# deepomicslab/PALACE

Measured on AMD Instinct MI355X. Metric: contigs/sec eref+generate_graph+matching, 1M-contig synth, 1/2/4/8 GPU, higher is better.
Workload: dtype u32

## Files before the change

include/palace_hip.h:

```cpp
#ifndef PALACE_HIP_H
#define PALACE_HIP_H

#include <stddef.h>
#include <stdint.h>

#ifdef __cplusplus
extern "C" {
#endif

#define PALACE_OK 0
#define PALACE_EINVAL (-1)
#define PALACE_EHIP (-2)
#define PALACE_ENOMEM (-3)
#define PALACE_ESTATE (-4)

typedef struct palace_ctx palace_ctx;

const char *palace_last_error(void);
const char *palace_version(void);

int palace_ctx_create(int device, palace_ctx **out);
int palace_ctx_create_prio(int device, int high_priority, palace_ctx **out);
int palace_ctx_create_on_stream(int device, void *hip_stream, palace_ctx **out);
int palace_ctx_destroy(palace_ctx *ctx);
// ... 21 lines not shown
int palace_eref_set_coder(palace_ctx *ctx, const uint8_t header400[400]);

int palace_eref_index_refs(palace_ctx *ctx, const uint8_t *d_bases, const int64_t *d_offsets,
                           int64_t n_refs, uint32_t *d_out, const int64_t *d_out_offsets);

int palace_eref_table_reset(palace_ctx *ctx);
int palace_eref_reserve(palace_ctx *ctx, int64_t total_bases);
int palace_eref_count_reads(palace_ctx *ctx, const uint8_t *d_bases, const int64_t *d_offsets,
                            int64_t n_reads, const uint8_t *d_keep, int64_t total_bases);

size_t palace_eref_packed_bytes(int64_t n_positions);
int palace_eref_pack_reads(palace_ctx *ctx, const uint8_t *d_bases, const int64_t *d_offsets, int64_t n_reads,
                           const uint8_t *d_keep, int64_t total_bases, uint32_t *d_p0, uint32_t *d_p1, uint32_t *d_u);
int palace_eref_count_reads_packed(palace_ctx *ctx, const uint32_t *d_p0, const uint32_t *d_p1, const uint32_t *d_u,
                                   int64_t n_positions, int64_t n_reads_hint);

int palace_eref_set_count_mode(palace_ctx *ctx, int mode, int64_t bucket_cap);
int palace_eref_set_key_buckets(palace_ctx *ctx, const uint32_t mask128[4]);
int palace_eref_set_option(palace_ctx *ctx, const char *name, int64_t value);

int palace_eref_scan_refs(palace_ctx *ctx, const uint8_t *d_bases, const int64_t *d_offsets,
                          int64_t n_refs, int64_t total_bases, int one_min, int three_min,
                          int32_t *d_rows);

typedef struct palace_eref_probe_index palace_eref_probe_index;
int palace_eref_probe_index_build(palace_ctx *ctx, const uint8_t *d_bases, const int64_t *d_offsets, int64_t n_refs,
                                  int64_t total_bases, palace_eref_probe_index **out);
int palace_eref_probe_index_free(palace_ctx *ctx, palace_eref_probe_index *ix);
int palace_eref_scan_refs_indexed(palace_ctx *ctx, const palace_eref_probe_index *ix, const uint8_t *d_bases,
                                  const int64_t *d_offsets, int64_t n_refs, int64_t total_bases, int one_min,
                                  int three_min, int32_t *d_rows);

int palace_eref_attach_probe_index(palace_ctx *ctx, const palace_eref_probe_index *ix);

int palace_eref_entry_layout(const palace_eref_probe_index *ix, size_t *counts_bytes, size_t *hits_bytes);
int palace_eref_entry_buffers_attach(palace_ctx *ctx, palace_eref_probe_index *ix, void *d_counts, void *d_hits);
int palace_eref_entry_buffers(const palace_eref_probe_index *ix, void **d_counts, void **d_hits);
int palace_eref_entry_hits_from_counts(palace_ctx *ctx, const palace_eref_probe_index *ix, const void *d_parts, int n_parts, size_t part_stride,
                                       size_t off, size_t bytes);
int palace_eref_entry_hits_complete(palace_ctx *ctx, const palace_eref_probe_index *ix, int64_t keys_counted);
int palace_eref_entry_counts_valid(const palace_ctx *ctx, const palace_eref_probe_index *ix);


int palace_eref_table_planes(palace_ctx *ctx, void **d_planes3, size_t *bytes_per_plane);
int palace_eref_table_attach(palace_ctx *ctx, void *const d_planes3[3]);
int palace_eref_table_invalidate(palace_ctx *ctx);
// ... 568 lines not shown
```

palace_amd/capi.py:

```python
from __future__ import annotations

import ctypes as C
import os
import subprocess

import numpy as np

_HERE = os.path.dirname(os.path.abspath(__file__))
SO_PATH = os.environ.get("PALACE_HIP_SO") or os.path.join(_HERE, "libpalace_hip.so")
_LIB = None


class PalaceError(RuntimeError):
    pass


def build(force: bool = False) -> str:
    args = ["make", "-C", os.path.join(_HERE, "csrc")]
    if force:
        subprocess.run(args + ["clean"], check=True, stdout=subprocess.DEVNULL)
    subprocess.run(args, check=True, stdout=subprocess.DEVNULL)
    return SO_PATH


# ... 105 lines not shown
    "palace_host_alloc": [C.c_void_p, C.c_size_t, C.POINTER(C.c_void_p)],
    "palace_host_free": [C.c_void_p, C.c_void_p],
    "palace_d2h_async": [C.c_void_p, C.c_void_p, C.c_void_p, C.c_size_t],
    "palace_h2d_async": [C.c_void_p, C.c_void_p, C.c_void_p, C.c_size_t],
    "palace_mark_wait": [C.c_void_p, C.c_int],
    "palace_mark_wait_for": [C.c_void_p, C.c_int, C.c_double],
    "palace_wait_for_mark": [C.c_void_p, C.c_void_p, C.c_int],
    "palace_timer_begin": [C.c_void_p],
    "palace_timer_end": [C.c_void_p, C.POINTER(C.c_float)],
    "palace_mark": [C.c_void_p, C.c_int],
    "palace_mark_elapsed": [C.c_void_p, C.c_int, C.c_int, C.POINTER(C.c_float)],
    "palace_eref_set_coder": [C.c_void_p, C.c_void_p],
    "palace_eref_index_refs": [C.c_void_p, C.c_void_p, C.c_void_p, C.c_int64, C.c_void_p, C.c_void_p],
    "palace_eref_table_reset": [C.c_void_p],
    "palace_eref_reserve": [C.c_void_p, C.c_int64],
    "palace_eref_count_reads": [C.c_void_p, C.c_void_p, C.c_void_p, C.c_int64, C.c_void_p, C.c_int64],
    "palace_eref_pack_reads": [C.c_void_p, C.c_void_p, C.c_void_p, C.c_int64, C.c_void_p, C.c_int64, C.c_void_p, C.c_void_p, C.c_void_p],
    "palace_eref_count_reads_packed": [C.c_void_p, C.c_void_p, C.c_void_p, C.c_void_p, C.c_int64, C.c_int64],
    "palace_eref_set_count_mode": [C.c_void_p, C.c_int, C.c_int64],
    "palace_eref_set_key_buckets": [C.c_void_p, C.c_void_p],
    "palace_eref_set_option": [C.c_void_p, C.c_char_p, C.c_int64],
    "palace_eref_scan_refs": [C.c_void_p, C.c_void_p, C.c_void_p, C.c_int64, C.c_int64, C.c_int, C.c_int,
                              C.c_void_p],
    "palace_eref_probe_index_build": [C.c_void_p, C.c_void_p, C.c_void_p, C.c_int64, C.c_int64, C.POINTER(C.c_void_p)],
    "palace_eref_attach_probe_index": [C.c_void_p, C.c_void_p],
    "palace_eref_entry_layout": [C.c_void_p, C.POINTER(C.c_size_t), C.POINTER(C.c_size_t)],
    "palace_eref_entry_buffers_attach": [C.c_void_p, C.c_void_p, C.c_void_p, C.c_void_p],
    "palace_eref_entry_buffers": [C.c_void_p, C.POINTER(C.c_void_p), C.POINTER(C.c_void_p)],
    "palace_eref_entry_hits_from_counts": [C.c_void_p, C.c_void_p, C.c_void_p, C.c_int, C.c_size_t, C.c_size_t, C.c_size_t],
    "palace_eref_entry_hits_complete": [C.c_void_p, C.c_void_p, C.c_int64],
    "palace_eref_entry_counts_valid": [C.c_void_p, C.c_void_p],
    "palace_eref_probe_index_free": [C.c_void_p, C.c_void_p],
    "palace_eref_scan_refs_indexed": [C.c_void_p, C.c_void_p, C.c_void_p, C.c_void_p, C.c_int64, C.c_int64, C.c_int, C.c_int,
                                      C.c_void_p],
    "palace_eref_table_planes": [C.c_void_p, C.POINTER(C.c_void_p), C.POINTER(C.c_size_t)],
    "palace_eref_table_attach": [C.c_void_p, C.POINTER(C.c_void_p)],
    "palace_eref_table_invalidate": [C.c_void_p],
    "palace_eref_table_merge_slices": [C.c_void_p, C.c_void_p, C.c_int, C.c_size_t, C.c_size_t],
    "palace_eref_table_merge_slices_packed": [C.c_void_p, C.c_void_p, C.c_int, C.c_size_t, C.c_size_t],
    "palace_eref_table_pack_low": [C.c_void_p, C.c_void_p],
    "palace_eref_plane_pack": [C.c_void_p, C.c_void_p, C.c_void_p, C.c_void_p, C.c_int64, C.c_void_p],
    "palace_eref_plane_unpack": [C.c_void_p, C.c_void_p, C.c_void_p, C.c_void_p, C.c_int64, C.c_void_p],
    "palace_eref_table_lookup": [C.c_void_p, C.c_void_p, C.c_int64, C.c_void_p],
    "palace_eref_table_popcounts": [C.c_void_p, C.POINTER(C.c_uint64)],
    "palace_graph_classify": [C.c_void_p, C.POINTER(BamCols), C.c_void_p, C.c_int32, C.c_void_p, C.c_void_p,
                              C.c_void_p, C.c_int64, C.POINTER(GraphParams), C.c_int64, C.c_void_p, C.c_void_p,
# ... 1811 lines not shown
```

palace_amd/csrc/eref_common.hpp:

```cpp
#pragma once
#include "common.hpp"

#ifdef PALACE_STAMPS
extern __device__ unsigned long long palace_stamp_buf[8 * 65536];
#define STAMP(arr, i) do { if (arr) (arr)[i] = __builtin_amdgcn_s_memrealtime(); } while (0)
#else
#define STAMP(arr, i) do { } while (0)
#endif

namespace palace {

struct BaseBits {
    bool p0, p1, p2, ok;
};

__device__ __forceinline__ BaseBits classify(uint32_t ch)
{
    const uint32_t x = ch & 0xDFu;
    const uint32_t d = x - 0x41u;
    const bool ok = d < 20u && ((0x80045u >> d) & 1u);
    const uint32_t c = x >> 1;
    return BaseBits{!(c & 1u), !(c & 2u), !((c ^ (c >> 1)) & 1u), ok};
}

// ... 178 lines not shown
static inline KeyBuckets ctx_buckets(const palace_ctx *ctx)
{
    KeyBuckets k;
    for (int i = 0; i < 4; i++) k.m[i] = ctx->key_buckets[i];
    return k;
}

constexpr size_t kTouchedBytes = 8192 + 256;
struct CountPlan {
    int64_t slab_bases_max = 0, n_slabs = 0, n_chunks = 0;
    DensityCaps caps1{}, caps2{};
    size_t cur1_bytes = 0, cur2_bytes = 0, buf1_bytes = 0, buf2_bytes = 0, words_bytes = 0;
    size_t total() const { return cur1_bytes + buf1_bytes + cur2_bytes + kTouchedBytes + 5 * words_bytes + buf2_bytes; }
};
constexpr int64_t kRegions = static_cast<int64_t>(kL1Buckets) * kL1Replicas;

struct CountBufs {
    unsigned int *cursor2 = nullptr, *touched = nullptr, *cursor1 = nullptr;
    unsigned long long *words = nullptr;
    uint32_t *buf1 = nullptr;
    uint16_t *buf2 = nullptr;
};

struct ScanBuffers {
    int64_t *tile_pre, *word_pre;
    uint64_t *any_w, *all_w, *good_w;
    uint32_t *any_p, *all_p;
    uint8_t *need, *active;
    uint8_t *hit_bytes;
    uint8_t *ehits[kSets];
    int64_t max_tiles, max_words;
};
int scan_buffers(palace_ctx *ctx, const int64_t *d_offsets, int64_t n_refs, int64_t total_bases, ScanBuffers *b, bool with_hit_bytes = false,
                 const size_t *ehits_bytes = nullptr);

}

struct palace_eref_probe_index {
    int64_t n_refs = 0, total_bases = 0;
    palace::CoderMasks masks{};
    unsigned long long n_entries[palace::kSets] = {0, 0, 0, 0};
    unsigned long long *first = nullptr;
    uint16_t *keys16[palace::kSets] = {nullptr, nullptr, nullptr, nullptr};
    uint32_t *eix[3] = {nullptr, nullptr, nullptr};
    uint32_t *pos_s = nullptr;
    uint8_t *ehits_own[palace::kSets] = {nullptr, nullptr, nullptr, nullptr};
    size_t ehits_own_bytes = 0;
    uint8_t *sent_bytes_own = nullptr;
    uint8_t *ecnt_own[palace::kSets] = {nullptr, nullptr, nullptr, nullptr};
    size_t entry_hits_bytes = 0;
    size_t set_at[palace::kSets] = {0, 0, 0, 0};
// ... 15 lines not shown
```

palace_amd/csrc/eref_scan.hip:

```cpp
#include "eref_common.hpp"

namespace palace {

__global__ __launch_bounds__(1024) void seq_prefix_kernel(const int64_t *__restrict__ offsets,
                                                          int64_t n, int64_t *__restrict__ tile_pre,
                                                          int64_t *__restrict__ word_pre)
{
    __shared__ int64_t s_t[1024], s_w[1024];
    const int t = threadIdx.x;
    const int64_t per = (n + 1023) / 1024;
    const int64_t a = min(n, t * per), b = min(n, a + per);
    int64_t st = 0, sw = 0;
    for (int64_t r = a; r < b; r++) {
        int64_t len = offsets[r + 1] - offsets[r];
        st += (len + kTilePos - 1) / kTilePos;
        sw += (len + 63) / 64;
    }
    s_t[t] = st;
    s_w[t] = sw;
    __syncthreads();
    for (int d = 1; d < 1024; d <<= 1) {
        int64_t vt = (t >= d) ? s_t[t - d] : 0, vw = (t >= d) ? s_w[t - d] : 0;
        __syncthreads();
        s_t[t] += vt;
        s_w[t] += vw;
        __syncthreads();
    }
    int64_t rt = s_t[t] - st, rw = s_w[t] - sw;
    for (int64_t r = a; r < b; r++) {
        int64_t len = offsets[r + 1] - offsets[r];
// ... 263 lines not shown
                at++;
            }
        }
        __syncthreads();
        const uint32_t n = min(n_list, static_cast<uint32_t>(kScatterList));
        const unsigned long long eb = base * 128;
        constexpr int kUn = 4;
        for (uint32_t j0 = threadIdx.x; j0 < n; j0 += kUn * kScatterThreads) {
            uint32_t p[kUn];
#pragma unroll
            for (int u = 0; u < kUn; u++) {
                const uint32_t j = j0 + u * kScatterThreads;
                p[u] = j < n ? pos[eb + list[j]] : ~0u;
            }
#pragma unroll
            for (int u = 0; u < kUn; u++)
                if (p[u] != ~0u) hit(p[u]);
        }
        __syncthreads();
    }
}

constexpr int kRefThreads = 1024;
__global__ __launch_bounds__(kRefThreads) void eref_need_kernel(const int64_t *__restrict__ offsets, int64_t n_refs,
                                                        const int64_t *__restrict__ word_pre,
                                                        const uint64_t *__restrict__ c0_words,
                                                        uint32_t *__restrict__ c0_pre, uint64_t *__restrict__ cand_words,
                                                        uint32_t *__restrict__ cand_pre, int three_min,
                                                        uint8_t *__restrict__ need, uint8_t *__restrict__ active,
                                                        int64_t r_lo, int64_t r_hi)
{
    const int64_t r = blockIdx.x;
    if (r >= n_refs) return;
    if (r < r_lo || r >= r_hi) { if (threadIdx.x == 0) active[r] = 0; return; }
    const int64_t len = offsets[r + 1] - offsets[r];
    const int64_t n_words = (len + 63) / 64, w0 = word_pre[r];
    const uint64_t *A = c0_words + w0;
    uint32_t *PA = c0_pre + w0, *PC = cand_pre + w0;
    uint64_t *C = cand_words + w0;
    const int t = threadIdx.x, lane = t & 63, wv = t >> 6;
    constexpr int kWaves = kRefThreads / 64;
    __shared__ uint32_t s_part[kWaves];
    __shared__ uint32_t carry;
    auto block_prefix = [&](const uint64_t *W, uint32_t *P) {
        if (t == 0) carry = 0;
        __syncthreads();
        for (int64_t base = 0; base < n_words; base += kRefThreads) {
            const int64_t w = base + t;
            const uint32_t c = (w < n_words) ? __popcll(W[w]) : 0;
            uint32_t inc = c;
#pragma unroll
            for (int d = 1; d < 64; d <<= 1) {
                uint32_t u = __shfl_up(inc, d);
                if (lane >= d) inc += u;
            }
            if (lane == 63) s_part[wv] = inc;
            __syncthreads();
            uint32_t o = carry;
            for (int k = 0; k < wv; k++) o += s_part[k];
            if (w < n_words) P[w] = o + inc - c;
            __syncthreads();
            if (t == kRefThreads - 1) carry = o + inc;
            __syncthreads();
        }
    };
    {
        bool dense = false;
        for (int64_t g = t; g * 8 < n_words; g += kRefThreads) {
            uint32_t c = 0;
#pragma unroll
            for (int k = 0; k < 8; k++) c += (g * 8 + k < n_words) ? __popcll(A[g * 8 + k]) : 0;
            dense |= 2 * static_cast<int>(c) >= three_min;
        }
        const bool live = __syncthreads_or(dense);
        if (!live) {
            if (t == 0) active[r] = 0;
            return;
        }
        if (t == 0) active[r] = 1;
    }
    block_prefix(A, PA);
    __threadfence_block();
    __syncthreads();
    for (int64_t w = wv; w < n_words; w += kWaves) {
        const int64_t j = w * 64 + lane;
        bool cand = false;
        if (j < len) {
            uint32_t c = prefix_count(A, PA, j);
            if (j >= 500) c -= prefix_count(A, PA, j - 500);
            cand = static_cast<int>(c) >= three_min;
        }
        const uint64_t g = __ballot(cand);
        if (lane == 0) C[w] = g;
    }
    __threadfence_block();
    __syncthreads();
    block_prefix(C, PC);
    __threadfence_block();
    __syncthreads();
    if (carry == 0) {
        if (t == 0) active[r] = 0;
        return;
    }
    for (int64_t w = t; w < n_words; w += kRefThreads) {
        const int64_t hi = min(len - 1, w * 64 + 63 + 499);
        uint32_t upto = prefix_count(C, PC, hi);
        uint32_t before = w ? prefix_count(C, PC, w * 64 - 1) : 0u;
        need[w0 + w] = upto > before;
    }
}

__global__ __launch_bounds__(kRefThreads) void eref_window_kernel(const int64_t *__restrict__ offsets,
                                                                  int64_t n_refs,
                                                                  const int64_t *__restrict__ word_pre,
                                                                  const uint64_t *__restrict__ any_words,
                                                                  const uint64_t *__restrict__ all_words,
                                                                  uint32_t *__restrict__ any_pre,
                                                                  uint32_t *__restrict__ all_pre,
                                                                  uint64_t *__restrict__ good_words,
                                                                  int one_min, int three_min,
                                                                  const uint8_t *__restrict__ active,
                                                                  int32_t *__restrict__ rows)
{
    const int64_t r = blockIdx.x;
    if (r >= n_refs) return;
    const int64_t len = offsets[r + 1] - offsets[r];
    if (!active[r]) {
        if (threadIdx.x == 0) { rows[4 * r + 0] = 0; rows[4 * r + 1] = 0; rows[4 * r + 2] = static_cast<int>(len); rows[4 * r + 3] = 0; }
        return;
    }
    const int64_t n_words = (len + 63) / 64, w0 = word_pre[r];
    const uint64_t *A = any_words + w0, *T = all_words + w0;
    uint32_t *PA = any_pre + w0, *PT = all_pre + w0;
    uint64_t *G = good_words + w0;
    const int t = threadIdx.x, lane = t & 63, wv = t >> 6;
    constexpr int kWaves = kRefThreads / 64;

    __shared__ uint32_t s_a[kWaves], s_t[kWaves];
    __shared__ uint32_t carry_a, carry_t;
    if (t == 0) { carry_a = 0; carry_t = 0; }
    __syncthreads();
    for (int64_t base = 0; base < n_words; base += kRefThreads) {
        int64_t w = base + t;
        uint32_t ca = (w < n_words) ? __popcll(A[w]) : 0, ct = (w < n_words) ? __popcll(T[w]) : 0;
        uint32_t ia = ca, it = ct;
#pragma unroll
        for (int d = 1; d < 64; d <<= 1) {
            uint32_t ua = __shfl_up(ia, d), ut = __shfl_up(it, d);
            if (lane >= d) { ia += ua; it += ut; }
        }
        if (lane == 63) { s_a[wv] = ia; s_t[wv] = it; }
        __syncthreads();
        uint32_t oa = carry_a, ot = carry_t;
        for (int k = 0; k < wv; k++) { oa += s_a[k]; ot += s_t[k]; }
        if (w < n_words) { PA[w] = oa + ia - ca; PT[w] = ot + it - ct; }
        __syncthreads();
        if (t == kRefThreads - 1) { carry_a = oa + ia; carry_t = ot + it; }
        __syncthreads();
    }
    __threadfence_block();
    __syncthreads();

    for (int64_t w = wv; w < n_words; w += kWaves) {
        int64_t j = w * 64 + lane;
        bool good = false;
        if (j < len) {
            uint32_t one = prefix_count(A, PA, j), three = prefix_count(T, PT, j);
            if (j >= 500) { one -= prefix_count(A, PA, j - 500); three -= prefix_count(T, PT, j - 500); }
            good = static_cast<int>(one) >= one_min && static_cast<int>(three) >= three_min;
        }
        uint64_t g = __ballot(good);
        if (lane == 0) G[w] = g;
    }
    __threadfence_block();
    __syncthreads();

    constexpr int kMaxEdges = 1024;
    __shared__ uint32_t edge[kMaxEdges];
    __shared__ unsigned int n_edge;
    if (t == 0) n_edge = 0;
    __syncthreads();
    for (int64_t w = t; w <= n_words; w += kRefThreads) {
        const uint64_t g = (w < n_words) ? G[w] : 0;
        const uint64_t prev_bit = w ? (G[w - 1] >> 63) : 0;
        uint64_t x = g ^ ((g << 1) | prev_bit);
        while (x) {
            const int b = __ffsll(static_cast<long long>(x)) - 1;
            x &= x - 1;
            const unsigned int at = atomicAdd(&n_edge, 1u);
            if (at < kMaxEdges) edge[at] = (static_cast<uint32_t>(w * 64 + b) << 1) | static_cast<uint32_t>((g >> b) & 1);
        }
    }
    __syncthreads();
    if (t == 0) {
        int frag = 0, el = 0, start = 0, prev_end = 0;
        const int ilen = static_cast<int>(len);
        auto on_edge = [&](int j, bool rising) {
            if (rising) {
                start = max(1, j - 1000);
            } else {
                int end = min(ilen, j + 1000);
                if (frag > 0 && start - prev_end < 500) { el += end - prev_end; }
                else { frag++; el += end - start; }
                prev_end = end;
            }
        };
        if (n_edge <= kMaxEdges) {
            const int n = static_cast<int>(n_edge);
            for (int i = 1; i < n; i++) {
                const uint32_t e = edge[i];
                int k = i - 1;
                while (k >= 0 && edge[k] > e) { edge[k + 1] = edge[k]; k--; }
                edge[k + 1] = e;
            }
            for (int i = 0; i < n; i++) on_edge(static_cast<int>(edge[i] >> 1), edge[i] & 1u);
        } else {
            uint64_t prev_bit = 0;
            for (int64_t w = 0; w <= n_words; w++) {
                uint64_t g = (w < n_words) ? G[w] : 0;
                uint64_t x = g ^ ((g << 1) | prev_bit);
                while (x) {
                    int b = __ffsll(static_cast<long long>(x)) - 1;
                    x &= x - 1;
                    on_edge(static_cast<int>(w * 64 + b), (g >> b) & 1);
                }
                prev_bit = g >> 63;
            }
        }
        rows[4 * r + 0] = frag;
        rows[4 * r + 1] = el;
        rows[4 * r + 2] = ilen;
        rows[4 * r + 3] = 0;
    }
}

}

using namespace palace;

extern "C" {

static int launch_prefix(palace_ctx *ctx, const int64_t *d_offsets, int64_t n, int64_t *tile_pre, int64_t *word_pre)
{
    hipLaunchKernelGGL(seq_prefix_kernel, dim3(1), dim3(1024), 0, ctx->stream, d_offsets, n, tile_pre, word_pre);
    PALACE_HIP_TRY(hipGetLastError());
    return PALACE_OK;
}

int palace_eref_index_refs(palace_ctx *ctx, const uint8_t *d_bases, const int64_t *d_offsets,
                           int64_t n_refs, uint32_t *d_out, const int64_t *d_out_offsets)
{
    PALACE_REQUIRE(ctx && n_refs >= 0, "bad argument");
    if (!ctx->coder_set) { set_error("palace_eref_index_refs: coder not set"); return PALACE_ESTATE; }
    if (n_refs == 0) return PALACE_OK;
    PALACE_REQUIRE(d_bases && d_offsets && d_out && d_out_offsets, "null device pointer");
    PALACE_HIP_TRY(hipSetDevice(ctx->device));
    int64_t h_off[2];
    PALACE_HIP_TRY(hipMemcpyAsync(&h_off[0], d_offsets, 8, hipMemcpyDeviceToHost, ctx->stream));
    PALACE_HIP_TRY(hipMemcpyAsync(&h_off[1], d_offsets + n_refs, 8, hipMemcpyDeviceToHost, ctx->stream));
    PALACE_HIP_TRY(hipStreamSynchronize(ctx->stream));
    int64_t total = h_off[1] - h_off[0];
    PALACE_REQUIRE(total >= 0, "offsets not ascending");
    size_t pre_bytes = align_up((n_refs + 1) * 8, 256);
    int rc = ensure_workspace(ctx, 2 * pre_bytes);
    if (rc) return rc;
    char *ws = static_cast<char *>(ctx->ws.ptr);
    int64_t *tile_pre = reinterpret_cast<int64_t *>(ws), *word_pre = reinterpret_cast<int64_t *>(ws + pre_bytes);
// ... 5 lines not shown
                       d_bases, d_offsets, n_refs, tile_pre, word_pre, ctx->masks,
                       static_cast<const uint32_t *>(nullptr), static_cast<uint64_t *>(nullptr),
                       static_cast<uint64_t *>(nullptr), d_out, d_out_offsets, static_cast<const uint8_t *>(nullptr),
                       static_cast<const uint8_t *>(nullptr));
    PALACE_HIP_TRY(hipGetLastError());
    return PALACE_OK;
}

}

namespace palace {
int scan_buffers(palace_ctx *ctx, const int64_t *d_offsets, int64_t n_refs, int64_t total_bases, ScanBuffers *b, bool with_hit_bytes,
                 const size_t *ehits_bytes)
{
    b->max_tiles = total_bases / kTilePos + n_refs;
    b->max_words = total_bases / 64 + n_refs + 1;
    PALACE_REQUIRE(b->max_tiles < (1ll << 31), "too many tiles for one launch");
    const size_t pre_bytes = align_up((n_refs + 1) * 8, 256);
    const size_t w64 = align_up(b->max_words * 8, 256), w32 = align_up(b->max_words * 4, 256);
    const size_t w8 = align_up(b->max_words, 256);
    const size_t hb = with_hit_bytes ? align_up(static_cast<size_t>(b->max_words) * (64 / kSentinelStride), 256) : 0;
    size_t eb[kSets] = {0, 0, 0, 0}, eb_all = 0;
    for (int k = 0; k < kSets; k++) { eb[k] = ehits_bytes && ehits_bytes[k] ? align_up(ehits_bytes[k] + 16, 256) : 0; eb_all += eb[k]; }
    int rc = ensure_workspace(ctx, 2 * pre_bytes + 3 * w64 + 2 * w32 + w8 + align_up(n_refs + 1, 256) + hb + eb_all);
    if (rc) return rc;
    char *ws = static_cast<char *>(ctx->ws.ptr);
    b->tile_pre = reinterpret_cast<int64_t *>(ws); ws += pre_bytes;
    b->word_pre = reinterpret_cast<int64_t *>(ws); ws += pre_bytes;
    b->any_w = reinterpret_cast<uint64_t *>(ws); ws += w64;
    b->all_w = reinterpret_cast<uint64_t *>(ws); ws += w64;
    b->good_w = reinterpret_cast<uint64_t *>(ws); ws += w64;
    b->any_p = reinterpret_cast<uint32_t *>(ws); ws += w32;
    b->all_p = reinterpret_cast<uint32_t *>(ws); ws += w32;
    b->need = reinterpret_cast<uint8_t *>(ws); ws += w8;
    b->active = reinterpret_cast<uint8_t *>(ws); ws += align_up(n_refs + 1, 256);
    b->hit_bytes = with_hit_bytes ? reinterpret_cast<uint8_t *>(ws) : nullptr; ws += hb;
    for (int k = 0; k < kSets; k++) { b->ehits[k] = eb[k] ? reinterpret_cast<uint8_t *>(ws) : nullptr; ws += eb[k]; }
    return launch_prefix(ctx, d_offsets, n_refs, b->tile_pre, b->word_pre);
}
}

namespace {
int scan_tail(palace_ctx *ctx, const ScanBuffers &b, const uint8_t *d_bases, const int64_t *d_offsets, int64_t n_refs,
              int one_min, int three_min, int32_t *d_rows)
{
    hipLaunchKernelGGL(eref_need_kernel, dim3(static_cast<unsigned>(n_refs)), dim3(kRefThreads), 0, ctx->stream, d_offsets,
                       n_refs, b.word_pre, b.any_w, b.any_p, b.good_w, b.all_p, three_min, b.need, b.active, static_cast<int64_t>(0), n_refs);
    PALACE_HIP_TRY(hipGetLastError());
    hipLaunchKernelGGL(eref_ref_kernel<0>, dim3(static_cast<unsigned>(b.max_tiles)), dim3(256), 0, ctx->stream,
                       d_bases, d_offsets, n_refs, b.tile_pre, b.word_pre, ctx->masks, ctx->plane[2], b.any_w,
                       b.all_w, static_cast<uint32_t *>(nullptr), static_cast<const int64_t *>(nullptr),
                       static_cast<const uint8_t *>(b.need), static_cast<const uint8_t *>(b.active));
    PALACE_HIP_TRY(hipGetLastError());
    hipLaunchKernelGGL(eref_window_kernel, dim3(static_cast<unsigned>(n_refs)), dim3(kRefThreads), 0, ctx->stream,
                       d_offsets, n_refs, b.word_pre, b.any_w, b.all_w, b.any_p, b.all_p, b.good_w, one_min, three_min,
                       static_cast<const uint8_t *>(b.active), d_rows);
    PALACE_HIP_TRY(hipGetLastError());
    return PALACE_OK;
}

int scan_args_ok(palace_ctx *ctx, const uint8_t *d_bases, const int64_t *d_offsets, int64_t n_refs, int64_t total_bases,
                 const int32_t *d_rows)
{
    PALACE_REQUIRE(ctx && n_refs >= 0 && total_bases >= 0, "bad argument");
    if (!ctx->coder_set) { set_error("scan_refs: coder not set"); return PALACE_ESTATE; }
    PALACE_REQUIRE(n_refs == 0 || (d_bases && d_offsets && d_rows), "null device pointer");
    PALACE_REQUIRE(n_refs < (1ll << 31), "too many refs for one launch");
    return PALACE_OK;
}

}

extern "C" {

int palace_eref_scan_refs(palace_ctx *ctx, const uint8_t *d_bases, const int64_t *d_offsets,
                          int64_t n_refs, int64_t total_bases, int one_min, int three_min,
                          int32_t *d_rows)
{
    int rc = scan_args_ok(ctx, d_bases, d_offsets, n_refs, total_bases, d_rows);
    if (rc || n_refs == 0) return rc;
    PALACE_REQUIRE(ctx->table.planes_readable(), kTableHoldsNothing);
    PALACE_HIP_TRY(hipSetDevice(ctx->device));
    rc = ensure_table(ctx);
    if (rc) return rc;
    ScanBuffers b;
    rc = scan_buffers(ctx, d_offsets, n_refs, total_bases, &b);
    if (rc) return rc;
    hipLaunchKernelGGL(eref_ref_kernel<2>, dim3(static_cast<unsigned>(b.max_tiles)), dim3(256), 0, ctx->stream,
                       d_bases, d_offsets, n_refs, b.tile_pre, b.word_pre, ctx->masks, ctx->plane[2], b.any_w,
                       b.all_w, static_cast<uint32_t *>(nullptr), static_cast<const int64_t *>(nullptr),
                       static_cast<const uint8_t *>(nullptr), static_cast<const uint8_t *>(nullptr));
    PALACE_HIP_TRY(hipGetLastError());
    return scan_tail(ctx, b, d_bases, d_offsets, n_refs, one_min, three_min, d_rows);
}

int palace_eref_scan_refs_indexed(palace_ctx *ctx, const palace_eref_probe_index *ix, const uint8_t *d_bases,
// ... 21 lines not shown
    const bool sent_done = ctx->table.sentinels_placed_for(ix);
    if (!sent_done) PALACE_HIP_TRY(hipMemsetAsync(b.hit_bytes, 0, static_cast<size_t>(b.max_words) * (64 / kSentinelStride), ctx->stream));
    ProbeSets sets{};
    for (int k = 0; k < kSets; k++) {
        const bool have = (fused >> k) & 1u;
        uint8_t *eh = have ? ix->ehits_own[k] : b.ehits[k];
        sets.s[k] = ProbeSet{ix->first + static_cast<size_t>(k) * (kIndexGroups + 1), ix->keys16[k], eh};
        if (!have) {
            sets.mask |= 1u << k;
            if (ix->ehits_bytes[k] >= 16) PALACE_HIP_TRY(hipMemsetAsync(eh + ix->ehits_bytes[k] - 16, 0, 16, ctx->stream));
        }
    }
    if (sets.mask) hipLaunchKernelGGL(eref_probe_sets_kernel, dim3(kBuckets), dim3(kProbeThreads), 0, ctx->stream, sets, ctx->plane[2]);
    const int64_t r_lo = std::min(ctx->scan_ref_lo, n_refs), r_hi = ctx->scan_ref_hi > 0 ? std::max(r_lo, std::min(ctx->scan_ref_hi, n_refs)) : n_refs;
    if (!sent_done)
        hipLaunchKernelGGL(eref_ehits_scatter_kernel, dim3(kCUs * 8), dim3(kScatterThreads), 0, ctx->stream,
                           reinterpret_cast<const uint4 *>(sets.s[kSentinelSet].ehits), static_cast<unsigned long long>(ix->ehits_bytes[kSentinelSet] / 16),
                           ix->pos_s, b.hit_bytes, static_cast<const int64_t *>(b.word_pre), r_lo, r_hi);
    hipLaunchKernelGGL(eref_sentinel_words_kernel, dim3(kCUs * 8), dim3(256), 0, ctx->stream,
                       reinterpret_cast<const uint4 *>(sent_done ? ix->sent_bytes_own : b.hit_bytes), b.max_words, b.any_w);
    PALACE_HIP_TRY(hipGetLastError());
    const int sentinel_min = std::max(0, 500 / kSentinelStride - 1 - (500 - three_min));
    hipLaunchKernelGGL(eref_need_kernel, dim3(static_cast<unsigned>(n_refs)), dim3(kRefThreads), 0, ctx->stream, d_offsets,
                       n_refs, b.word_pre, b.any_w, b.any_p, b.good_w, b.all_p, sentinel_min, b.need, b.active, r_lo, r_hi);
    GatherArgs ga{};
    for (int c = 0; c < 3; c++) { ga.eix[c] = ix->eix[c]; ga.ehits[c] = sets.s[c].ehits; }
    const dim3 tiles(static_cast<unsigned>(b.max_tiles));
    const uint8_t *need = b.need, *active = b.active;
    const bool sparse_table = ctx->table.known_sparse();
    if (sparse_table) {
        hipLaunchKernelGGL(eref_gather_hits_kernel<0>, tiles, dim3(256), 0, ctx->stream, d_offsets, n_refs, b.tile_pre, b.word_pre, ga, need, active,
                           b.any_w, b.all_w);
    } else {
        hipLaunchKernelGGL(eref_gather_hits_kernel<1>, tiles, dim3(256), 0, ctx->stream, d_offsets, n_refs, b.tile_pre, b.word_pre, ga, need, active,
                           b.any_w, b.all_w);
        hipLaunchKernelGGL(eref_need_kernel, dim3(static_cast<unsigned>(n_refs)), dim3(kRefThreads), 0, ctx->stream, d_offsets,
                           n_refs, b.word_pre, b.any_w, b.any_p, b.good_w, b.all_p, three_min, b.need, b.active, r_lo, r_hi);
        hipLaunchKernelGGL(eref_gather_hits_kernel<2>, tiles, dim3(256), 0, ctx->stream, d_offsets, n_refs, b.tile_pre, b.word_pre, ga, need, active,
                           b.any_w, b.all_w);
    }
    hipLaunchKernelGGL(eref_window_kernel, dim3(static_cast<unsigned>(n_refs)), dim3(kRefThreads), 0, ctx->stream,
                       d_offsets, n_refs, b.word_pre, b.any_w, b.all_w, b.any_p, b.all_p, b.good_w, one_min, three_min,
                       static_cast<const uint8_t *>(b.active), d_rows);
    PALACE_HIP_TRY(hipGetLastError());
    return PALACE_OK;
}

}
```

Before: 112.8 million.

## Split eref window scan into per-segment work items with stitch pass

The per-reference window kernel, one 1024-thread block per contig, is replaced by a segment-parallel design. The need kernel appends (ref, segment) work items for active references and writes rows for inactive ones. A persistent window kernel computes a per-segment run summary using a halo of words, and a stitch kernel merges the summaries per reference into frag/el rows. The need kernel also stages its prefix arrays in LDS for short references. The goal is to remove the load imbalance and heavy per-ref block cost of the old window kernel, at the price of extra kernels, atomics and workspace.

```diff
diff --git a/include/palace_hip.h b/include/palace_hip.h
--- a/include/palace_hip.h
+++ b/include/palace_hip.h
@@ -67,6 +67,7 @@
 int palace_eref_scan_refs(palace_ctx *ctx, const uint8_t *d_bases, const int64_t *d_offsets,
                           int64_t n_refs, int64_t total_bases, int one_min, int three_min,
                           int32_t *d_rows);
+int palace_eref_scan_segment_positions(void);
 
 typedef struct palace_eref_probe_index palace_eref_probe_index;
 int palace_eref_probe_index_build(palace_ctx *ctx, const uint8_t *d_bases, const int64_t *d_offsets, int64_t n_refs,
diff --git a/palace_amd/capi.py b/palace_amd/capi.py
--- a/palace_amd/capi.py
+++ b/palace_amd/capi.py
@@ -151,6 +151,7 @@
     "palace_eref_set_option": [C.c_void_p, C.c_char_p, C.c_int64],
     "palace_eref_scan_refs": [C.c_void_p, C.c_void_p, C.c_void_p, C.c_int64, C.c_int64, C.c_int, C.c_int,
                               C.c_void_p],
+    "palace_eref_scan_segment_positions": [],
     "palace_eref_probe_index_build": [C.c_void_p, C.c_void_p, C.c_void_p, C.c_int64, C.c_int64, C.POINTER(C.c_void_p)],
     "palace_eref_attach_probe_index": [C.c_void_p, C.c_void_p],
     "palace_eref_entry_layout": [C.c_void_p, C.POINTER(C.c_size_t), C.POINTER(C.c_size_t)],
diff --git a/palace_amd/csrc/eref_common.hpp b/palace_amd/csrc/eref_common.hpp
--- a/palace_amd/csrc/eref_common.hpp
+++ b/palace_amd/csrc/eref_common.hpp
@@ -224,11 +224,15 @@
     uint16_t *buf2 = nullptr;
 };
 
+constexpr int kSegSummaryInts = 8;
 struct ScanBuffers {
     int64_t *tile_pre, *word_pre;
     uint64_t *any_w, *all_w, *good_w;
     uint32_t *any_p, *all_p;
     uint8_t *need, *active;
+    int32_t *seg_sum;
+    unsigned int *n_work;
+    uint32_t *work;
     uint8_t *hit_bytes;
     uint8_t *ehits[kSets];
     int64_t max_tiles, max_words;
diff --git a/palace_amd/csrc/eref_scan.hip b/palace_amd/csrc/eref_scan.hip
--- a/palace_amd/csrc/eref_scan.hip
+++ b/palace_amd/csrc/eref_scan.hip
@@ -4,8 +4,9 @@
 
 __global__ __launch_bounds__(1024) void seq_prefix_kernel(const int64_t *__restrict__ offsets,
                                                           int64_t n, int64_t *__restrict__ tile_pre,
-                                                          int64_t *__restrict__ word_pre)
-{
+                                                          int64_t *__restrict__ word_pre, unsigned int *__restrict__ n_work)
+{
+    if (threadIdx.x == 0 && n_work) *n_work = 0;
     __shared__ int64_t s_t[1024], s_w[1024];
     const int t = threadIdx.x;
     const int64_t per = (n + 1023) / 1024;
@@ -315,22 +316,27 @@
 }
 
 constexpr int kRefThreads = 1024;
+constexpr int kNeedLdsWords = 2048;
 __global__ __launch_bounds__(kRefThreads) void eref_need_kernel(const int64_t *__restrict__ offsets, int64_t n_refs,
                                                         const int64_t *__restrict__ word_pre,
                                                         const uint64_t *__restrict__ c0_words,
                                                         uint32_t *__restrict__ c0_pre, uint64_t *__restrict__ cand_words,
                                                         uint32_t *__restrict__ cand_pre, int three_min,
                                                         uint8_t *__restrict__ need, uint8_t *__restrict__ active,
-                                                        int64_t r_lo, int64_t r_hi)
+                                                        int64_t r_lo, int64_t r_hi,
+                                                        int32_t *__restrict__ rows,
+                                                        const int64_t *__restrict__ tile_pre, unsigned int *__restrict__ n_work,
+                                                        uint2 *__restrict__ work)
 {
     const int64_t r = blockIdx.x;
     if (r >= n_refs) return;
-    if (r < r_lo || r >= r_hi) { if (threadIdx.x == 0) active[r] = 0; return; }
     const int64_t len = offsets[r + 1] - offsets[r];
+    auto inactive = [&]() {
+        if (threadIdx.x == 0) { active[r] = 0; rows[4 * r + 0] = 0; rows[4 * r + 1] = 0; rows[4 * r + 2] = static_cast<int>(len); rows[4 * r + 3] = 0; }
+    };
+    if (r < r_lo || r >= r_hi) { inactive(); return; }
     const int64_t n_words = (len + 63) / 64, w0 = word_pre[r];
     const uint64_t *A = c0_words + w0;
-    uint32_t *PA = c0_pre + w0, *PC = cand_pre + w0;
-    uint64_t *C = cand_words + w0;
     const int t = threadIdx.x, lane = t & 63, wv = t >> 6;
     constexpr int kWaves = kRefThreads / 64;
     __shared__ uint32_t s_part[kWaves];
@@ -367,11 +373,20 @@
         }
         const bool live = __syncthreads_or(dense);
         if (!live) {
-            if (t == 0) active[r] = 0;
+            inactive();
             return;
         }
         if (t == 0) active[r] = 1;
     }
+    __shared__ uint64_t l_a[kNeedLdsWords], l_c[kNeedLdsWords];
+    __shared__ uint32_t l_pa[kNeedLdsWords], l_pc[kNeedLdsWords];
+    const bool in_lds = n_words <= kNeedLdsWords;
+    if (in_lds) {
+        for (int64_t w = t; w < n_words; w += kRefThreads) l_a[w] = A[w];
+        A = l_a;
+    }
+    uint32_t *PA = in_lds ? l_pa : c0_pre + w0, *PC = in_lds ? l_pc : cand_pre + w0;
+    uint64_t *C = in_lds ? l_c : cand_words + w0;
     block_prefix(A, PA);
     __threadfence_block();
     __syncthreads();
@@ -392,7 +407,7 @@
     __threadfence_block();
     __syncthreads();
     if (carry == 0) {
-        if (t == 0) active[r] = 0;
+        inactive();
         return;
     }
     for (int64_t w = t; w < n_words; w += kRefThreads) {
@@ -401,129 +416,152 @@
         uint32_t before = w ? prefix_count(C, PC, w * 64 - 1) : 0u;
         need[w0 + w] = upto > before;
     }
-}
-
-__global__ __launch_bounds__(kRefThreads) void eref_window_kernel(const int64_t *__restrict__ offsets,
-                                                                  int64_t n_refs,
+    __shared__ unsigned int list_at;
+    const int64_t n_seg = tile_pre[r + 1] - tile_pre[r];
+    if (t == 0) list_at = atomicAdd(n_work, static_cast<unsigned int>(n_seg));
+    __syncthreads();
+    for (int64_t sgm = t; sgm < n_seg; sgm += kRefThreads) work[list_at + sgm] = uint2{static_cast<uint32_t>(r), static_cast<uint32_t>(sgm)};
+}
+
+constexpr int kSegWords = kTileChunks, kSegHalo = 8, kSegLds = kSegHalo + kSegWords, kSegThreads = 256;
+static_assert(kSegHalo * 64 >= 501 && kSegLds <= 64, "good[j] of the position in front of a segment reaches 500 further back; a wave scans the words");
+struct alignas(16) SegSummary {
+    int32_t frag, el;
+    int32_t first_fall, first_rise;
+    int32_t last_fall, last_rise;
+    int32_t pad[2];
+};
+static_assert(sizeof(SegSummary) == 4 * kSegSummaryInts, "ScanBuffers::seg_sum");
+
+__device__ __forceinline__ void add_run(int &frag, int &el, int ilen, int rise, int fall, int prev_fall)
+{
+    const int start = max(1, rise - 1000), end = min(ilen, fall + 1000), prev_end = min(ilen, prev_fall + 1000);
+    if (prev_fall >= 0 && start - prev_end < 500) { el += end - prev_end; }
+    else { frag++; el += end - start; }
+}
+
+__device__ __forceinline__ void window_segment(const int64_t r, const int64_t seg, const int64_t *__restrict__ offsets,
+                                               const int64_t *__restrict__ tile_pre, const int64_t *__restrict__ word_pre,
+                                               const uint64_t *__restrict__ any_words, const uint64_t *__restrict__ all_words,
+                                               int one_min, int three_min, SegSummary *__restrict__ seg_sum)
+{
+    const int64_t len = offsets[r + 1] - offsets[r], n_words = (len + 63) / 64, w0 = word_pre[r];
+    const int64_t tile = tile_pre[r] + seg;
+    const int64_t ws = seg * kSegWords - kSegHalo;
+    const int t = threadIdx.x, lane = t & 63, wv = t >> 6;
+    __shared__ uint64_t s_w[2][kSegLds], s_g[kSegWords + 1];
+    __shared__ uint32_t s_p[2][kSegLds];
+
+    if (wv < 2) {
+        const uint64_t *W = (wv ? all_words : any_words) + w0;
+        const int64_t w = ws + lane;
+        const uint64_t v = (lane < kSegLds && w >= 0 && w < n_words) ? W[w] : 0ull;
+        const uint32_t c = __popcll(v);
+        uint32_t inc = c;
+#pragma unroll
+        for (int d = 1; d < 64; d <<= 1) {
+            const uint32_t u = __shfl_up(inc, d);
+            if (lane >= d) inc += u;
+        }
+        if (lane < kSegLds) { s_w[wv][lane] = v; s_p[wv][lane] = inc - c; }
+    }
+    __syncthreads();
+
+    auto upto = [&](int ch, int64_t j) {
+        const int k = static_cast<int>((j >> 6) - ws), b = static_cast<int>(j & 63);
+        const uint64_t mask = (b == 63) ? ~0ull : ((2ull << b) - 1);
+        return s_p[ch][k] + static_cast<uint32_t>(__popcll(s_w[ch][k] & mask));
+    };
+    for (int lw = kSegHalo - 1 + wv; lw < kSegLds; lw += kSegThreads / 64) {
+        const int64_t j = (ws + lw) * 64 + lane;
+        bool good = false;
+        if (j >= 0 && j < len && (lw >= kSegHalo || lane == 63)) {
+            uint32_t one = upto(0, j), three = upto(1, j);
+            if (j >= 500) { one -= upto(0, j - 500); three -= upto(1, j - 500); }
+            good = static_cast<int>(one) >= one_min && static_cast<int>(three) >= three_min;
+        }
+        const uint64_t g = __ballot(good);
+        if (lane == 0) s_g[lw - (kSegHalo - 1)] = g;
+    }
+    __syncthreads();
+    if (wv != 0) return;
+
+    const int ilen = static_cast<int>(len);
+    const uint64_t g = lane < kSegWords ? s_g[lane + 1] : 0ull, prev_bit = lane < kSegWords ? s_g[lane] >> 63 : 0ull;
+    uint64_t x = g ^ ((g << 1) | prev_bit);
+    const int base = static_cast<int>(seg * kTilePos) + lane * 64;
+    const uint64_t xr = x & g, xf = x & ~g;
+    int last_r = xr ? base + 63 - __clzll(static_cast<long long>(xr)) : -1, last_f = xf ? base + 63 - __clzll(static_cast<long long>(xf)) : -1;
+#pragma unroll
+    for (int d = 1; d < 64; d <<= 1) {
+        const int ur = __shfl_up(last_r, d), uf = __shfl_up(last_f, d);
+        if (lane >= d) { last_r = max(last_r, ur); last_f = max(last_f, uf); }
+    }
+    int cur_r = __shfl_up(last_r, 1), cur_f = __shfl_up(last_f, 1);
+    if (lane == 0) { cur_r = -1; cur_f = -1; }
+    int frag = 0, el = 0, first_fall = -1, first_rise = -1;
+    while (x) {
+        const int b = __ffsll(static_cast<long long>(x)) - 1;
+        x &= x - 1;
+        const int j = base + b;
+        if ((g >> b) & 1) { cur_r = j; continue; }
+        if (cur_f < 0) { first_fall = j; first_rise = cur_r; }
+        else add_run(frag, el, ilen, cur_r, j, cur_f);
+        cur_f = j;
+    }
+#pragma unroll
+    for (int d = 32; d >= 1; d >>= 1) { frag += __shfl_xor(frag, d); el += __shfl_xor(el, d); }
+    const uint64_t has_first = __ballot(first_fall >= 0);
+    const int src = has_first ? __ffsll(static_cast<long long>(has_first)) - 1 : 0;
+    first_fall = __shfl(first_fall, src);
+    first_rise = __shfl(first_rise, src);
+    last_r = __shfl(last_r, 63);
+    last_f = __shfl(last_f, 63);
+
+    if (lane == 0) seg_sum[tile] = SegSummary{frag, el, first_fall, first_rise, last_f, last_r, {0, 0}};
+}
+
+__global__ __launch_bounds__(kSegThreads) void eref_stitch_kernel(const int64_t *__restrict__ offsets, const int64_t *__restrict__ tile_pre,
+                                                                  const unsigned int *__restrict__ n_work, const uint2 *__restrict__ work,
+                                                                  const SegSummary *__restrict__ seg_sum, int32_t *__restrict__ rows)
+{
+    const unsigned int n = *n_work, lane = threadIdx.x & 63, n_waves = gridDim.x * (kSegThreads / 64);
+    for (unsigned int i = (blockIdx.x * kSegThreads + threadIdx.x) >> 6; i < n; i += n_waves) {
+        const uint2 rs = work[i];
+        if (rs.y != 0) continue;
+        const int64_t r = rs.x, n_seg = tile_pre[r + 1] - tile_pre[r];
+        const int ilen = static_cast<int>(offsets[r + 1] - offsets[r]);
+        const SegSummary *S = seg_sum + tile_pre[r];
+        int frag = 0, el = 0, cur_r = -1, cur_f = -1;
+        for (int64_t s0 = 0; s0 < n_seg; s0 += 64) {
+            SegSummary m{0, 0, -1, -1, -1, -1, {0, 0}};
+            if (s0 + lane < n_seg) m = S[s0 + lane];
+            const int cnt = static_cast<int>(min(static_cast<int64_t>(64), n_seg - s0));
+            for (int k = 0; k < cnt; k++) {
+                const int ff = __shfl(m.first_fall, k), fr = __shfl(m.first_rise, k), lf = __shfl(m.last_fall, k), lr = __shfl(m.last_rise, k);
+                if (ff >= 0) add_run(frag, el, ilen, fr >= 0 ? fr : cur_r, ff, cur_f);
+                frag += __shfl(m.frag, k);
+                el += __shfl(m.el, k);
+                if (lf >= 0) cur_f = lf;
+                if (lf >= 0 || lr >= 0) cur_r = lr > lf ? lr : -1;
+            }
+        }
+        if (cur_r >= 0) add_run(frag, el, ilen, cur_r, ilen, cur_f);
+        if (lane == 0) { rows[4 * r + 0] = frag; rows[4 * r + 1] = el; rows[4 * r + 2] = ilen; rows[4 * r + 3] = 0; }
+    }
+}
+
+__global__ __launch_bounds__(kSegThreads) void eref_window_kernel(const int64_t *__restrict__ offsets, const int64_t *__restrict__ tile_pre,
                                                                   const int64_t *__restrict__ word_pre,
-                                                                  const uint64_t *__restrict__ any_words,
-                                                                  const uint64_t *__restrict__ all_words,
-                                                                  uint32_t *__restrict__ any_pre,
-                                                                  uint32_t *__restrict__ all_pre,
-                                                                  uint64_t *__restrict__ good_words,
-                                                                  int one_min, int three_min,
-                                                                  const uint8_t *__restrict__ active,
-                                                                  int32_t *__restrict__ rows)
-{
-    const int64_t r = blockIdx.x;
-    if (r >= n_refs) return;
-    const int64_t len = offsets[r + 1] - offsets[r];
-    if (!active[r]) {
-        if (threadIdx.x == 0) { rows[4 * r + 0] = 0; rows[4 * r + 1] = 0; rows[4 * r + 2] = static_cast<int>(len); rows[4 * r + 3] = 0; }
-        return;
-    }
-    const int64_t n_words = (len + 63) / 64, w0 = word_pre[r];
-    const uint64_t *A = any_words + w0, *T = all_words + w0;
-    uint32_t *PA = any_pre + w0, *PT = all_pre + w0;
-    uint64_t *G = good_words + w0;
-    const int t = threadIdx.x, lane = t & 63, wv = t >> 6;
-    constexpr int kWaves = kRefThreads / 64;
-
-    __shared__ uint32_t s_a[kWaves], s_t[kWaves];
-    __shared__ uint32_t carry_a, carry_t;
-    if (t == 0) { carry_a = 0; carry_t = 0; }
-    __syncthreads();
-    for (int64_t base = 0; base < n_words; base += kRefThreads) {
-        int64_t w = base + t;
-        uint32_t ca = (w < n_words) ? __popcll(A[w]) : 0, ct = (w < n_words) ? __popcll(T[w]) : 0;
-        uint32_t ia = ca, it = ct;
-#pragma unroll
-        for (int d = 1; d < 64; d <<= 1) {
-            uint32_t ua = __shfl_up(ia, d), ut = __shfl_up(it, d);
-            if (lane >= d) { ia += ua; it += ut; }
-        }
-        if (lane == 63) { s_a[wv] = ia; s_t[wv] = it; }
+                                                                  const uint64_t *__restrict__ any_words, const uint64_t *__restrict__ all_words,
+                                                                  int one_min, int three_min, const unsigned int *__restrict__ n_work,
+                                                                  const uint2 *__restrict__ work, SegSummary *__restrict__ seg_sum)
+{
+    const unsigned int n = *n_work;
+    for (unsigned int i = blockIdx.x; i < n; i += gridDim.x) {
+        const uint2 rs = work[i];
+        window_segment(rs.x, rs.y, offsets, tile_pre, word_pre, any_words, all_words, one_min, three_min, seg_sum);
         __syncthreads();
-        uint32_t oa = carry_a, ot = carry_t;
-        for (int k = 0; k < wv; k++) { oa += s_a[k]; ot += s_t[k]; }
-        if (w < n_words) { PA[w] = oa + ia - ca; PT[w] = ot + it - ct; }
-        __syncthreads();
-        if (t == kRefThreads - 1) { carry_a = oa + ia; carry_t = ot + it; }
-        __syncthreads();
-    }
-    __threadfence_block();
-    __syncthreads();
-
-    for (int64_t w = wv; w < n_words; w += kWaves) {
-        int64_t j = w * 64 + lane;
-        bool good = false;
-        if (j < len) {
-            uint32_t one = prefix_count(A, PA, j), three = prefix_count(T, PT, j);
-            if (j >= 500) { one -= prefix_count(A, PA, j - 500); three -= prefix_count(T, PT, j - 500); }
-            good = static_cast<int>(one) >= one_min && static_cast<int>(three) >= three_min;
-        }
-        uint64_t g = __ballot(good);
-        if (lane == 0) G[w] = g;
-    }
-    __threadfence_block();
-    __syncthreads();
-
-    constexpr int kMaxEdges = 1024;
-    __shared__ uint32_t edge[kMaxEdges];
-    __shared__ unsigned int n_edge;
-    if (t == 0) n_edge = 0;
-    __syncthreads();
-    for (int64_t w = t; w <= n_words; w += kRefThreads) {
-        const uint64_t g = (w < n_words) ? G[w] : 0;
-        const uint64_t prev_bit = w ? (G[w - 1] >> 63) : 0;
-        uint64_t x = g ^ ((g << 1) | prev_bit);
-        while (x) {
-            const int b = __ffsll(static_cast<long long>(x)) - 1;
-            x &= x - 1;
-            const unsigned int at = atomicAdd(&n_edge, 1u);
-            if (at < kMaxEdges) edge[at] = (static_cast<uint32_t>(w * 64 + b) << 1) | static_cast<uint32_t>((g >> b) & 1);
-        }
-    }
-    __syncthreads();
-    if (t == 0) {
-        int frag = 0, el = 0, start = 0, prev_end = 0;
-        const int ilen = static_cast<int>(len);
-        auto on_edge = [&](int j, bool rising) {
-            if (rising) {
-                start = max(1, j - 1000);
-            } else {
-                int end = min(ilen, j + 1000);
-                if (frag > 0 && start - prev_end < 500) { el += end - prev_end; }
-                else { frag++; el += end - start; }
-                prev_end = end;
-            }
-        };
-        if (n_edge <= kMaxEdges) {
-            const int n = static_cast<int>(n_edge);
-            for (int i = 1; i < n; i++) {
-                const uint32_t e = edge[i];
-                int k = i - 1;
-                while (k >= 0 && edge[k] > e) { edge[k + 1] = edge[k]; k--; }
-                edge[k + 1] = e;
-            }
-            for (int i = 0; i < n; i++) on_edge(static_cast<int>(edge[i] >> 1), edge[i] & 1u);
-        } else {
-            uint64_t prev_bit = 0;
-            for (int64_t w = 0; w <= n_words; w++) {
-                uint64_t g = (w < n_words) ? G[w] : 0;
-                uint64_t x = g ^ ((g << 1) | prev_bit);
-                while (x) {
-                    int b = __ffsll(static_cast<long long>(x)) - 1;
-                    x &= x - 1;
-                    on_edge(static_cast<int>(w * 64 + b), (g >> b) & 1);
-                }
-                prev_bit = g >> 63;
-            }
-        }
-        rows[4 * r + 0] = frag;
-        rows[4 * r + 1] = el;
-        rows[4 * r + 2] = ilen;
-        rows[4 * r + 3] = 0;
     }
 }
 
@@ -533,9 +571,9 @@
 
 extern "C" {
 
-static int launch_prefix(palace_ctx *ctx, const int64_t *d_offsets, int64_t n, int64_t *tile_pre, int64_t *word_pre)
-{
-    hipLaunchKernelGGL(seq_prefix_kernel, dim3(1), dim3(1024), 0, ctx->stream, d_offsets, n, tile_pre, word_pre);
+static int launch_prefix(palace_ctx *ctx, const int64_t *d_offsets, int64_t n, int64_t *tile_pre, int64_t *word_pre, unsigned int *n_work = nullptr)
+{
+    hipLaunchKernelGGL(seq_prefix_kernel, dim3(1), dim3(1024), 0, ctx->stream, d_offsets, n, tile_pre, word_pre, n_work);
     PALACE_HIP_TRY(hipGetLastError());
     return PALACE_OK;
 }
@@ -587,7 +625,9 @@
     const size_t hb = with_hit_bytes ? align_up(static_cast<size_t>(b->max_words) * (64 / kSentinelStride), 256) : 0;
     size_t eb[kSets] = {0, 0, 0, 0}, eb_all = 0;
     for (int k = 0; k < kSets; k++) { eb[k] = ehits_bytes && ehits_bytes[k] ? align_up(ehits_bytes[k] + 16, 256) : 0; eb_all += eb[k]; }
-    int rc = ensure_workspace(ctx, 2 * pre_bytes + 3 * w64 + 2 * w32 + w8 + align_up(n_refs + 1, 256) + hb + eb_all);
+    const size_t sb = align_up(static_cast<size_t>(b->max_tiles) * kSegSummaryInts * 4, 256);
+    const size_t wb = align_up(static_cast<size_t>(b->max_tiles) * 8, 256);
+    int rc = ensure_workspace(ctx, 2 * pre_bytes + 3 * w64 + 2 * w32 + w8 + align_up(n_refs + 1, 256) + sb + 256 + wb + hb + eb_all);
     if (rc) return rc;
     char *ws = static_cast<char *>(ctx->ws.ptr);
     b->tile_pre = reinterpret_cast<int64_t *>(ws); ws += pre_bytes;
@@ -599,9 +639,12 @@
     b->all_p = reinterpret_cast<uint32_t *>(ws); ws += w32;
     b->need = reinterpret_cast<uint8_t *>(ws); ws += w8;
     b->active = reinterpret_cast<uint8_t *>(ws); ws += align_up(n_refs + 1, 256);
+    b->seg_sum = reinterpret_cast<int32_t *>(ws); ws += sb;
+    b->n_work = reinterpret_cast<unsigned int *>(ws); ws += 256;
+    b->work = reinterpret_cast<uint32_t *>(ws); ws += wb;
     b->hit_bytes = with_hit_bytes ? reinterpret_cast<uint8_t *>(ws) : nullptr; ws += hb;
     for (int k = 0; k < kSets; k++) { b->ehits[k] = eb[k] ? reinterpret_cast<uint8_t *>(ws) : nullptr; ws += eb[k]; }
-    return launch_prefix(ctx, d_offsets, n_refs, b->tile_pre, b->word_pre);
+    return launch_prefix(ctx, d_offsets, n_refs, b->tile_pre, b->word_pre, b->n_work);
 }
 }
 
@@ -610,16 +653,20 @@
               int one_min, int three_min, int32_t *d_rows)
 {
     hipLaunchKernelGGL(eref_need_kernel, dim3(static_cast<unsigned>(n_refs)), dim3(kRefThreads), 0, ctx->stream, d_offsets,
-                       n_refs, b.word_pre, b.any_w, b.any_p, b.good_w, b.all_p, three_min, b.need, b.active, static_cast<int64_t>(0), n_refs);
+                       n_refs, b.word_pre, b.any_w, b.any_p, b.good_w, b.all_p, three_min, b.need, b.active, static_cast<int64_t>(0), n_refs,
+                       d_rows, b.tile_pre, b.n_work, reinterpret_cast<uint2 *>(b.work));
     PALACE_HIP_TRY(hipGetLastError());
     hipLaunchKernelGGL(eref_ref_kernel<0>, dim3(static_cast<unsigned>(b.max_tiles)), dim3(256), 0, ctx->stream,
                        d_bases, d_offsets, n_refs, b.tile_pre, b.word_pre, ctx->masks, ctx->plane[2], b.any_w,
                        b.all_w, static_cast<uint32_t *>(nullptr), static_cast<const int64_t *>(nullptr),
                        static_cast<const uint8_t *>(b.need), static_cast<const uint8_t *>(b.active));
     PALACE_HIP_TRY(hipGetLastError());
-    hipLaunchKernelGGL(eref_window_kernel, dim3(static_cast<unsigned>(n_refs)), dim3(kRefThreads), 0, ctx->stream,
-                       d_offsets, n_refs, b.word_pre, b.any_w, b.all_w, b.any_p, b.all_p, b.good_w, one_min, three_min,
-                       static_cast<const uint8_t *>(b.active), d_rows);
+    hipLaunchKernelGGL(eref_window_kernel, dim3(static_cast<unsigned>(std::min<int64_t>(b.max_tiles, kCUs * 8))), dim3(kSegThreads), 0, ctx->stream,
+                       d_offsets, b.tile_pre, b.word_pre, b.any_w, b.all_w, one_min, three_min, static_cast<const unsigned int *>(b.n_work),
+                       reinterpret_cast<const uint2 *>(b.work), reinterpret_cast<SegSummary *>(b.seg_sum));
+    hipLaunchKernelGGL(eref_stitch_kernel, dim3(static_cast<unsigned>(std::min<int64_t>(b.max_tiles, kCUs * 8))), dim3(kSegThreads), 0, ctx->stream,
+                       d_offsets, b.tile_pre, static_cast<const unsigned int *>(b.n_work), reinterpret_cast<const uint2 *>(b.work),
+                       reinterpret_cast<const SegSummary *>(b.seg_sum), d_rows);
     PALACE_HIP_TRY(hipGetLastError());
     return PALACE_OK;
 }
@@ -637,6 +684,8 @@
 }
 
 extern "C" {
+
+int palace_eref_scan_segment_positions(void) { return kTilePos; }
 
 int palace_eref_scan_refs(palace_ctx *ctx, const uint8_t *d_bases, const int64_t *d_offsets,
                           int64_t n_refs, int64_t total_bases, int one_min, int three_min,
@@ -704,7 +753,8 @@
     PALACE_HIP_TRY(hipGetLastError());
     const int sentinel_min = std::max(0, 500 / kSentinelStride - 1 - (500 - three_min));
     hipLaunchKernelGGL(eref_need_kernel, dim3(static_cast<unsigned>(n_refs)), dim3(kRefThreads), 0, ctx->stream, d_offsets,
-                       n_refs, b.word_pre, b.any_w, b.any_p, b.good_w, b.all_p, sentinel_min, b.need, b.active, r_lo, r_hi);
+                       n_refs, b.word_pre, b.any_w, b.any_p, b.good_w, b.all_p, sentinel_min, b.need, b.active, r_lo, r_hi, d_rows,
+                       b.tile_pre, b.n_work, reinterpret_cast<uint2 *>(b.work));
     GatherArgs ga{};
     for (int c = 0; c < 3; c++) { ga.eix[c] = ix->eix[c]; ga.ehits[c] = sets.s[c].ehits; }
     const dim3 tiles(static_cast<unsigned>(b.max_tiles));
@@ -716,14 +766,19 @@
     } else {
         hipLaunchKernelGGL(eref_gather_hits_kernel<1>, tiles, dim3(256), 0, ctx->stream, d_offsets, n_refs, b.tile_pre, b.word_pre, ga, need, active,
                            b.any_w, b.all_w);
+        PALACE_HIP_TRY(hipMemsetAsync(b.n_work, 0, sizeof(unsigned int), ctx->stream));
         hipLaunchKernelGGL(eref_need_kernel, dim3(static_cast<unsigned>(n_refs)), dim3(kRefThreads), 0, ctx->stream, d_offsets,
-                           n_refs, b.word_pre, b.any_w, b.any_p, b.good_w, b.all_p, three_min, b.need, b.active, r_lo, r_hi);
+                           n_refs, b.word_pre, b.any_w, b.any_p, b.good_w, b.all_p, three_min, b.need, b.active, r_lo, r_hi, d_rows,
+                           b.tile_pre, b.n_work, reinterpret_cast<uint2 *>(b.work));
         hipLaunchKernelGGL(eref_gather_hits_kernel<2>, tiles, dim3(256), 0, ctx->stream, d_offsets, n_refs, b.tile_pre, b.word_pre, ga, need, active,
                            b.any_w, b.all_w);
     }
-    hipLaunchKernelGGL(eref_window_kernel, dim3(static_cast<unsigned>(n_refs)), dim3(kRefThreads), 0, ctx->stream,
-                       d_offsets, n_refs, b.word_pre, b.any_w, b.all_w, b.any_p, b.all_p, b.good_w, one_min, three_min,
-                       static_cast<const uint8_t *>(b.active), d_rows);
+    hipLaunchKernelGGL(eref_window_kernel, dim3(static_cast<unsigned>(std::min<int64_t>(b.max_tiles, kCUs * 8))), dim3(kSegThreads), 0, ctx->stream,
+                       d_offsets, b.tile_pre, b.word_pre, b.any_w, b.all_w, one_min, three_min, static_cast<const unsigned int *>(b.n_work),
+                       reinterpret_cast<const uint2 *>(b.work), reinterpret_cast<SegSummary *>(b.seg_sum));
+    hipLaunchKernelGGL(eref_stitch_kernel, dim3(static_cast<unsigned>(std::min<int64_t>(b.max_tiles, kCUs * 8))), dim3(kSegThreads), 0, ctx->stream,
+                       d_offsets, b.tile_pre, static_cast<const unsigned int *>(b.n_work), reinterpret_cast<const uint2 *>(b.work),
+                       reinterpret_cast<const SegSummary *>(b.seg_sum), d_rows);
     PALACE_HIP_TRY(hipGetLastError());
     return PALACE_OK;
 }
```

Result: no change. 112.8 million (-0.0%).
